# pweigmann/harmonic-power-flow

Hardware: AMD Instinct MI355X
Metric: NR iterations/sec + ms/iter, 1 000-bus x 25-harmonic feeder; |dV| vs reference (higher is better)
Workload: dtype f64

## Files before the change

### harmonic-power-flow_amd/csrc/hpf_block.hip

```cpp
#include <algorithm>
#include <chrono>
#include <complex>
#include <cstdio>
#include <cstdlib>
#include <rocsolver/rocsolver.h>
#include <thread>

#include "hpf_internal.hpp"
#include "hpf_gj.hpp"
#include "hpf_blk_jobs.hpp"
#include "hpf_blk_invert_mfma.hpp"
#include "hpf_gj_dense.hpp"
#include "hpf_gj_mfma.hpp"

using namespace hpf;

#ifdef HPF_FACTOR_STAMPS
#define HPF_STAMP_DECL long long st0 = 0, st1 = 0, st2 = 0, st3 = 0, st4 = 0, st5 = 0, st6 = 0
#define HPF_STAMP(v) \
    if (ablate & 16) v = __builtin_amdgcn_s_memtime()
#else
#define HPF_STAMP_DECL
#define HPF_STAMP(v)
#endif

namespace {

// ... 745 lines not shown
#endif
        const int i = bid - nb_sl - nb_lf;
        back_q_body<B>(i % n_gj, i / n_gj, M, T, gj_nodes, b, N, Nc, active, Zall, wall, xall, (double*)nullptr, Hall, Minv, lfK, lfS, s0);
    }
}

template <int B>
int launch_level_back(hpf_handle* h, const TreeDev& T, const int* sl_nodes, int n_sl, const int* lf_nodes, int n_lf, const int* gj_nodes, int n_gj,
                      const int* active) {
    const Tree& tr = active_tree(h);
    const unsigned ytiles = (unsigned)((h->cur_S + LB_SB - 1) / LB_SB);
#if HPF_BATCH_XCD
    const unsigned grid = (unsigned)(((n_sl + 7) / 8) * 8 + ((n_lf + 7) / 8) * 8) * ytiles + (unsigned)n_gj * (unsigned)h->cur_S;
#else
    const unsigned grid = (unsigned)(n_sl + n_lf) * ytiles + (unsigned)n_gj * (unsigned)h->cur_S;
#endif
    if ((unsigned)(n_sl + n_lf) * ytiles + (unsigned)n_gj * (unsigned)h->cur_S == 0) return HPF_OK;
    hipLaunchKernelGGL((k_level_back<B>), dim3(grid), dim3(256), 0, h->cur_stream, h->M, T, sl_nodes, n_sl, lf_nodes, n_lf, gj_nodes, n_gj, 2 * h->Hn,
                       h->N, h->Nc, active, h->cur_S, h->d_Z, h->d_w, h->d_x, h->d_H, tr.d_Minv, tr.d_lbimg, tr.d_sbimg, tr.d_lzimg, h->d_lfK, h->d_lfS,
                       h->cur_s0);
    return launch_status(h);
}

__global__ __launch_bounds__(256) void k_border_prepare(int n, int Hn, int Bst, int b, int r, int v0, int vfirst, const int* __restrict__ tb_bus,
                                                        int n_tb, const double* __restrict__ g, cplx* __restrict__ U, cplx* __restrict__ E,
                                                        cplx* __restrict__ I0, double* __restrict__ fb) {
    const int j = blockIdx.y, v = vfirst + j;
    const size_t dst = (size_t)(v0 + j);
    const int t = blockIdx.x * 256 + threadIdx.x;
    if (t < n * Hn) {
        U[dst * n * Hn + t] = U[(size_t)r * n * Hn + t];
        E[dst * n * Hn + t] = E[(size_t)r * n * Hn + t];
    }
    if (t < n) I0[dst * n + t] = I0[(size_t)r * n + t];
    if (t < n * Bst) {
        double val = 0.0;
        if (v == 0) {
            val = fb[(size_t)r * n * Bst + t];
            if (g) {
                const int bus = t / Bst, l = t - bus * Bst;
                if (l < b)
                    for (int a = 0; a < n_tb; ++a)
                        if (tb_bus[a] == bus) val -= g[a * b + l];
            }
        } else {
            const int a = (v - 1) / b, l = (v - 1) - a * b;
// ... 55 lines not shown
    if (h->gj_mode != 1 || !h->sw.fuse_levels || (BW != 12 && BW != 28 && BW != 52)) return false;
    return BW == 52 || level_batched(h, T, l, nullptr) > 0;
}

bool tree_levels_fused(hpf_handle* h) {
    if (h->solver != HPF_SOLVER_BLOCK_TREE) return false;
    const Tree& T = active_tree(h);
    const int BW = wave_block_size(2 * h->Hn);
    if (T.n_levels == 0) return false;
    for (int l = 0; l < T.n_levels; ++l)
        if (T.lvl_ptr[l + 1] > T.lvl_ptr[l] && !level_is_fused(h, T, l, BW)) return false;
    return true;
}

Tree& active_tree(hpf_handle* h) { return (h->has_ctree && h->gj_mode == 1) ? h->ctree : h->tree; }

static void tree_free_one(Tree& T);
static void tree_free_one_fwd(Tree& T) { tree_free_one(T); }
static void tree_free_one(Tree& T) {
    void* ptrs[] = {T.d_parent, T.d_lvl_nodes, T.d_dep_nodes, T.d_child_ptr, T.d_child, T.d_e_up, T.d_e_dn,
                    T.d_child_mid, T.d_lin, T.d_lin_ptr, T.d_lin_post, T.d_all_ptr, T.d_all_post, T.d_fdesc, T.d_child3,
                    T.d_bdesc, T.d_dchild, T.d_chain_ptr, T.d_chain_nodes, T.d_chain_ch, T.d_Minv, T.d_lrec, T.d_crec, T.d_cnode, T.d_arec,
                    T.d_lzrec, T.d_lzimg, T.d_lbimg, T.d_bleaf, T.d_bsleaf, T.d_bsleaf_dep, T.d_sbimg, T.d_lbrec, T.d_lbptr, T.d_lb2rec, T.d_lb2x, T.d_lb2ptr, T.d_lb2cptr, T.d_lb2clist,
                    T.d_comp_child};
    for (void* p : ptrs)
        if (p) hipFree(p);
}

void tree_free(hpf_handle* h) {
    tree_free_one(h->tree);
    tree_free_one(h->ctree);
    void* bp[] = {h->d_tb_bus, h->d_tb_ptr, h->d_tb_adj, h->d_bM, h->d_brhs, h->d_bipiv, h->d_binfo, h->d_bM0, h->d_brhs0,
                  h->d_sel_P, h->d_sel_pidx, h->d_sel_toff, h->d_sel_S, h->d_sel_Z, h->d_sel_Up, h->d_sel_W, h->d_sel_X, h->d_sel_tie, h->d_sel_jobs,
                  h->d_sel_hl, h->d_sel_slot, h->d_sel_cptr, h->d_sel_clist, h->d_sel_dw, h->d_bB, h->d_bgj_jobs,
                  h->d_sel_bM, h->d_sel_rhs, h->d_sel_g, h->d_sel_res, h->d_sel_info};
    for (void* q2 : bp)
        if (q2) hipFree(q2);
}

int tree_alloc_scenarios(hpf_handle* h) {
    const int bw = wave_block_size(2 * h->Hn);
    const size_t b = bw ? (size_t)bw : 2 * (size_t)h->Hn, S = h->S_alloc, n = h->n;
    hipError_t e;
    const size_t ct = bw ? (size_t)(((bw + 16) / 16) * ((bw + 16) / 16) * 256) : 0;
    if ((e = hipMalloc((void**)&h->d_Z, sizeof(double) * S * n * (b * b > ct ? b * b : ct))) != hipSuccess ||
        (e = hipMalloc((void**)&h->d_w, sizeof(double) * S * n * b)) != hipSuccess ||
        (e = hipMalloc((void**)&h->d_x, sizeof(double) * S * n * b)) != hipSuccess ||
// ... 175 lines not shown
            case 28: r = factor_level<28>(h, T, td, l, active); break;
            case 52: r = factor_level<52>(h, T, td, l, active); break;
            case 100:
                if (h->gj_mode == 1) {
                    r = launch_factor_q<100>(h, td, T.d_fdesc + FDESC * (size_t)T.lvl_ptr[l], cnt, active, T.lvl_all_leaf[l] != 0);
                    break;
                }
                [[fallthrough]];
            default: r = factor_level_generic(h, td, T.d_lvl_nodes + T.lvl_ptr[l], cnt, active);
        }
        if (r) return r;
    }
    return HPF_OK;
}

static bool back_is_fused(const hpf_handle* h, const Tree& T, int BW) {
    bool fused = h->sw.fuse_back && h->cur_S <= h->sw.fuse_back_max && h->sw.leafbatch && h->has_ctree && h->gj_mode == 1 && BW == 52 &&
                 (int)T.bsl_dep_ptr.size() == T.n_depths + 1 && (int)T.bleaf_dep_ptr.size() == T.n_depths + 1 && (int)T.dep_nleaf.size() >= T.n_depths;
    for (int dl = 1; fused && dl < T.n_depths; ++dl)
        fused = T.bsl_dep_ptr[dl + 1] - T.bsl_dep_ptr[dl] + T.bleaf_dep_ptr[dl + 1] - T.bleaf_dep_ptr[dl] == T.dep_nleaf[dl];
    return fused && T.bsl_dep_ptr[1] == 0 && T.bleaf_dep_ptr[1] == 0;
}

template <int BW>
static int back_depth(hpf_handle* h, const Tree& T, const TreeDev& td, int dl, int nlb, const int* active) {
    const int cnt = T.dep_ptr[dl + 1] - T.dep_ptr[dl];
    if (h->gj_mode != 1) return launch_back_w<BW>(h, td, T.d_dep_nodes + T.dep_ptr[dl], cnt, active);
    return cnt > nlb ? launch_back_q<BW>(h, td, T.d_bdesc + 4 * (size_t)(T.dep_ptr[dl] + nlb), cnt - nlb, active) : HPF_OK;
}

template <int BW>
static int back_batched(hpf_handle* h, const Tree& T, const int* active) {
    for (size_t gi = 0; gi + 1 < T.bsleaf_ptr.size() && T.n_bsleaf > 0; ++gi) {
        const int b0 = T.bsleaf_ptr[gi], cnt = T.bsleaf_ptr[gi + 1] - b0;
        if (cnt <= 0) continue;
        if (int r = launch_sleaf_back_batch<BW>(h, T.d_bsleaf + 8 * (size_t)b0, cnt, active)) return r;
    }
    return T.n_bleaf > 0 ? launch_leaf_back_batch<BW>(h, T.d_bleaf, T.n_bleaf, active) : HPF_OK;
}

static int back_sweep(hpf_handle* h, const Tree& T, const TreeDev& td, const int* active, int Bst) {
    ScopedTimer tb(h, T_BACK);
    const int BW = wave_block_size(2 * h->Hn);
    const bool fused_back = back_is_fused(h, T, BW);
    for (int dl = 0; dl < T.n_depths; ++dl) {
        const int cnt = T.dep_ptr[dl + 1] - T.dep_ptr[dl];
        if (cnt == 0) continue;
        const int* nodes = T.d_dep_nodes + T.dep_ptr[dl];
        const int nlb = (h->sw.leafbatch && h->has_ctree && dl > 0 && dl < (int)T.dep_nleaf.size()) ? T.dep_nleaf[dl] : 0;
        int r = HPF_OK;
        if (fused_back) {
            const int n_sl = dl > 0 ? T.bsl_dep_ptr[dl + 1] - T.bsl_dep_ptr[dl] : 0, n_lf = dl > 0 ? T.bleaf_dep_ptr[dl + 1] - T.bleaf_dep_ptr[dl] : 0;
            r = launch_level_back<52>(h, td, T.d_bsleaf_dep + 8 * (size_t)T.bsl_dep_ptr[dl], n_sl, T.d_bleaf + 4 * (size_t)T.bleaf_dep_ptr[dl], n_lf,
                                      T.d_bdesc + 4 * (size_t)(T.dep_ptr[dl] + nlb), cnt - nlb, active);
        } else {
            switch (BW) {
                case 12: r = back_depth<12>(h, T, td, dl, nlb, active); break;
                case 28: r = back_depth<28>(h, T, td, dl, nlb, active); break;
                case 52: r = back_depth<52>(h, T, td, dl, nlb, active); break;
                case 100:
                    if (h->gj_mode == 1) {
                        r = launch_back_q<100>(h, td, T.d_bdesc + 4 * (size_t)T.dep_ptr[dl], cnt, active);
                        break;
                    }
                    [[fallthrough]];
                default:
// ... 715 lines not shown
```

### harmonic-power-flow_amd/csrc/hpf_internal.hpp

```cpp
#pragma once
#include <hip/hip_runtime.h>
#include <rocblas/rocblas.h>
#include <stdint.h>

#include <stdlib.h>
#include <string.h>

#include <string>
#include <vector>

#include "../../include/hpf.h"
#include "hpf_assembly.hpp"
#include "hpf_switches.hpp"

namespace hpf {

enum LinForm {
    LIN_ROOTS = 0,
    LIN_BUNDLE,
    LIN_TREE,
    LIN_LEVELS
};

enum { T_MISMATCH = 0, T_JACOBIAN = 1, T_SOLVE = 2, T_UPDATE = 3, T_BACK = 4, T_GJ = 5, T_GJ_DEV = 6, T_COUNT = 7 };

struct TimedSpan {
    int which;
    hipEvent_t e0, e1;
};

struct Tree {
    int n_levels = 0;
    int n_depths = 0;
    std::vector<int> parent;
    std::vector<int> lvl_ptr;
    std::vector<int> lvl_nodes;
    std::vector<int> dep_ptr;
    std::vector<int> dep_nodes;
    std::vector<int> child_ptr;
    std::vector<int> child;
    std::vector<int> child_mid;
    std::vector<int> lin;
    std::vector<int> lin_ptr;
    std::vector<int> lin_post;
    std::vector<int> all_ptr, all_post;
    int n_lin_roots = 0;
    int n_dense = 0;
    int* d_parent = nullptr;
    int* d_lvl_nodes = nullptr;
    int* d_dep_nodes = nullptr;
    int* d_child_ptr = nullptr;
    int* d_child = nullptr;
// ... 33 lines not shown
    int* d_cnode = nullptr;
    int n_all_heights = 0;
    std::vector<int> ah_ptr;
    int* d_arec = nullptr;
    std::vector<int> lvl_all_leaf;
    std::vector<int> toff_tab;
    std::vector<char> plain_gj;
    int n_cleaf = 0;
    double* d_Minv = nullptr;
    int n_lazy_parents = 0, n_lazy_leaves = 0;
    int n_lazy_level0 = 0;
    std::vector<int> lvl_nbatch;
    std::vector<int> dep_nleaf;
    std::vector<int> dep_nskip;
    int census[8] = {0, 0, 0, 0, 0, 0, 0, 0};
    std::vector<int> bsleaf_ptr;
    int n_bsleaf = 0;
    int* d_bsleaf = nullptr;
    double* d_sbimg = nullptr;
    std::vector<int> bsl_dep_ptr, bleaf_dep_ptr;
    int* d_bsleaf_dep = nullptr;
    int n_bleaf = 0;
    int* d_bleaf = nullptr;
    double* d_lbimg = nullptr;
    int* d_lzrec = nullptr;
    double* d_lzimg = nullptr;
    int n_comp = 0;
    std::vector<int> comp_v, comp_c;
    int* d_comp_child = nullptr;
    double plan_ms = 0.0;
    double flops_per_solve = 0.0;
    double flops_factor = 0.0;
    double bytes_back = 0.0;
    double bytes_factor = 0.0;
    double flops_gj = 0.0, bytes_gj = 0.0;
    int n_gj_launches = 0;
};

}

struct hpf_handle {
    hpf::Switches sw;
    hpf::Model M{};
    int n = 0, m = 0, c = 0, Hn = 0, nnz = 0, n_dev = 0, coupled = 0, solver = 0, device = 0;
    int S_max = 0, S = 0;
    int S_alloc = 0;
// ... 169 lines not shown
```

### harmonic-power-flow_amd/csrc/hpf_quad.hpp

```cpp
#pragma once

template <int CTRL>
__device__ __forceinline__ double dpp_f64(double v) {
    int lo = __double2loint(v), hi = __double2hiint(v);
    lo = __builtin_amdgcn_update_dpp(lo, lo, CTRL, 0xf, 0xf, false);
    hi = __builtin_amdgcn_update_dpp(hi, hi, CTRL, 0xf, 0xf, false);
    return __hiloint2double(hi, lo);
}

__device__ __forceinline__ double row_sum16(double v) {
    v += dpp_f64<0xB1>(v);
    v += dpp_f64<0x4E>(v);
    v += dpp_f64<0x141>(v);
    v += dpp_f64<0x140>(v);
    return v;
}

__device__ __forceinline__ Blk2 blk_current(cplx y, cplx Uj, cplx Ej) {
    Blk2 b;
    b.dV = cmul_unf(y, Ej);
    b.dA = cmul_unf(cmulj(y), Uj);
    return b;
}
__device__ __forceinline__ Blk2 blk_current_diag(cplx y, cplx U, cplx E, cplx yn, bool nonlinear) {
// ... 1278 lines not shown
        __shared__ cplx ynl[(B / 2) * (B / 2)];
        __shared__ double tab[(B / 2) * 8], dgb[RP * 3], cc[NT][RP * 3], panel[2][NT * 64], wl[2][16], pv[2][16], gl[NT * 32], hl[NT * 32];
        __shared__ double slb[B <= 52 ? 2 * B * 10 + 200 + 4 : 1];
        lds.ynl = ynl; lds.tab = tab; lds.dgb = dgb; lds.cc = cc; lds.panel = panel; lds.wl = wl; lds.pv = pv; lds.gl = gl; lds.hl = hl; lds.slb = slb;
        lds.gl2 = lds.hl2 = lds.pbuf = nullptr;
    } else {
        __shared__ __attribute__((aligned(16))) double smem[factor_q_lds<B>()];
        lds = FqLds<B>::carve(smem);
    }
    int bx = blockIdx.x, by = blockIdx.y;
#if HPF_LEAF_XCD
    if constexpr (LEAF) {
        const unsigned id = blockIdx.x, t = id >> 3, S_ = gridDim.y == 1 ? leaf_S : 1u;
        by = (int)(t % S_);
        bx = (int)((t / S_) * 8u + (id & 7u));
        if (bx >= leaf_count) return;
    }
#endif
    factor_q_body<B, LEAF>(lds, bx, by, M, T, nodes, b, N, Nc, active, Uall, Eall, fall, Zall, wall, linAall, Call, Hall, I0all, chG,
                           chH, chD, chy, Minv, lfK, lfS, dbg, ablate, s0, pivflag, piv_limit, tstamp);
}

template <int B>
__device__ __forceinline__ void back_q_body(
    const int bx_, const int by_, const Model& M, const TreeDev& T, const int* __restrict__ nodes, int b, int N, int Nc, const int* __restrict__ active,
    const double* __restrict__ Zall, const double* __restrict__ wall, double* __restrict__ xall, double* __restrict__ step,
    const double* __restrict__ Hall, const double* __restrict__ Minv, const double* __restrict__ lfK,
    const double* __restrict__ lfS, int s0) {
    constexpr int NT = (B + 16) / 16;
    constexpr size_t CT = (size_t)NT * NT * 256;
    const int s = active ? active[by_ + s0] : (int)by_ + s0;
    if (s < 0) return;
    const int4 kp = reinterpret_cast<const int4*>(nodes)[bx_];
    const int k = kp.x, par = kp.y, cleaf = kp.z;
    const int crole = kp.w >> 28, cinfo = kp.w & 0x0fffffff;
    const int tid = threadIdx.x, lane = tid & 63, lg = lane >> 4, jj = lane & 15;
    const int wv = __builtin_amdgcn_readfirstlane(tid >> 6);
    const int n = M.n, c = M.c, Hn = M.Hn;
    double* xs = xall + (size_t)s * n * B;
    constexpr int RP = 16 * NT > 64 ? 16 * NT : 64;
    __shared__ double part[NT][RP];
    __shared__ double mcl[RP * 2], zl[RP];
    double x = 0.0;
    if (tid < B) x = wall[((size_t)s * n + k) * B + tid];
    if (par >= 0) {
        double zr[NT * 4];
        if (cleaf) {
            TileIO<B>::load(Minv + (size_t)(cleaf - 1) * CT, wv, lg, jj, zr);
        } else {
            TileIO<B>::load(Zall + ((size_t)s * n + k) * CT, wv, lg, jj, zr);
        }
        const int col = 16 * wv + jj, p = col >> 1, t1 = col & 1;
        double tv = 0.0;
        if (crole == 2) {
            double hr[NT * 4];
            TileIO<B>::load(T.cF + (((size_t)s * T.n_comp + cinfo) * 3 + 2) * CT, wv, lg, jj, hr);
            const double xpc = col < b ? xs[(size_t)par * B + col] : 0.0;
#pragma unroll
            for (int e = 0; e < NT * 4; ++e)
                if (16 * (e >> 2) + 4 * (e & 3) < B) {
                    const double r = row_sum16(hr[e] * xpc);
                    if (jj == 0) part[wv][16 * (e >> 2) + lg + 4 * (e & 3)] = r;
                }
            __syncthreads();
            if (tid < B) {
                double acc = part[0][tid];
#pragma unroll
                for (int w2 = 1; w2 < NT; ++w2) acc += part[w2][tid];
                zl[tid] = acc;
            }
            __syncthreads();
            tv = col < b ? zl[col] : 0.0;
            __syncthreads();
        } else if (col < b) {
            const double* hk = Hall + ((size_t)s * n + k) * Hn * 4 + p * 4 + t1 * 2;
            const double* xp = xs + (size_t)par * B;
            tv = fma(hk[1], xp[2 * p + 1], hk[0] * xp[2 * p]);
            if (crole == 1) {
                const double* h2 = T.cH2 + ((size_t)s * T.n_comp + cinfo) * Hn * 4 + p * 4 + t1 * 2;
                const double* xc = xs + (size_t)T.comp_child[cinfo] * B;
                tv += fma(h2[1], xc[2 * p + 1], h2[0] * xc[2 * p]);
            }
        }
        if (cleaf && tid < 2) zl[tid] = tv;
        const double tvs = (cleaf && col < 2) ? 0.0 : tv;
        __builtin_amdgcn_sched_barrier(0);
#pragma unroll
        for (int e = 0; e < NT * 4; ++e)
            if (16 * (e >> 2) + 4 * (e & 3) < B) {
                const double r = row_sum16(zr[e] * tvs);
                if (jj == 0) part[wv][16 * (e >> 2) + lg + 4 * (e & 3)] = r;
                if (cleaf && wv == 0 && jj < 2) mcl[(16 * (e >> 2) + lg + 4 * (e & 3)) * 2 + jj] = zr[e];
            }
        __syncthreads();
        double acc = 0.0;
        if (tid < B) {
            acc = part[0][tid];
#pragma unroll
            for (int w2 = 1; w2 < NT; ++w2) acc += part[w2][tid];
        }
        if (cleaf) {
            double t0 = 0.0, t1v = 0.0;
            if (tid < B) {
                t0 = zl[0];
                t1v = zl[1];
            }
            __syncthreads();
            if (tid < 2) zl[tid] = acc + (tid == 0 ? t0 : t1v);
            __syncthreads();
            if (tid < B) {
                const double* kk = lfK + ((size_t)s * n + k) * 12;
                const double u0 = fma(kk[1], zl[1], kk[0] * zl[0]), u1 = fma(kk[3], zl[1], kk[2] * zl[0]);
                const double c0r = tid < 2 ? (tid == 0 ? 1.0 : 0.0) : mcl[tid * 2];
                const double c1r = tid < 2 ? (tid == 1 ? 1.0 : 0.0) : mcl[tid * 2 + 1];
                acc = fma(c1r, u1, fma(c0r, u0, tid < 2 ? 0.0 : acc));
            }
            __syncthreads();
            if (tid < B) zl[tid] = acc;
            __syncthreads();
            if (tid < B) {
                const double* si = lfS + (((size_t)s * n + k) * Hn + (tid >> 1)) * 4 + 2 * (tid & 1);
                acc = (tid >> 1) < Hn ? fma(si[1], zl[tid | 1], si[0] * zl[tid & ~1]) : acc;
            }
        }
        if (tid < B) x -= acc;
    }
    if (tid < B) {
        xs[(size_t)k * B + tid] = x;
        if (step && tid < b) {
            const int kst = (tid >> 1) * n + k;
            double* st = step + (size_t)s * N;
            if (tid & 1) {
                if (kst >= c) st[Nc + kst - c] = x;
            } else {
                if (kst >= 1) st[kst - 1] = x;
            }
        }
    }
}

template <int B>
__global__ __launch_bounds__(64 * ((B + 16) / 16)) void k_back_q(
    Model M, TreeDev T, const int* __restrict__ nodes, int b, int N, int Nc, const int* __restrict__ active,
    const double* __restrict__ Zall, const double* __restrict__ wall, double* __restrict__ xall, double* __restrict__ step,
    const double* __restrict__ Hall, const double* __restrict__ Minv, const double* __restrict__ lfK,
    const double* __restrict__ lfS, int s0) {
    back_q_body<B>(blockIdx.x, blockIdx.y, M, T, nodes, b, N, Nc, active, Zall, wall, xall, step, Hall, Minv, lfK, lfS, s0);
}

// ... 31 lines not shown
```

### harmonic-power-flow_amd/csrc/hpf_switches.hpp

```cpp
#pragma once
#include <stdlib.h>
#include <string.h>

#include <string>

namespace hpf {

struct Switches {
    bool tree_info = false;
    bool border_info = false;
    bool queue_info = false;
    std::string tree_dump;
    int debug_ablate = 0;
    int gj_mode = 1;
    int n_groups = 4;
    bool leafbatch = true;
    bool fuse_levels = true;
    bool fuse_back = true;
    int fuse_back_max = 32;
    int border_slot_cap = 1024;
    bool lintree = true;
    bool linbundle = true;
    bool chainbundle = true;
    int sleaf = 2;
    bool slback = true;
    bool sllazy = true;
    bool slnest = true;
    int lazy = 2;
    bool compress = true;
    bool mesh_sel = true;
    int border_gj = 96;
    bool border_gj_mfma = true;
    double border_pivlim = 1e3;
    double mesh_batch_gb = 48.0;
    bool mesh_batch_gb_given = false;
};

inline Switches parse_switches(const char* options, bool env_opt_in) {
    const std::string opts = options ? options : "";
    auto find = [&](const char* name) -> const char* {
        const size_t ln = strlen(name);
        size_t pos = 0;
// ... 3 lines not shown
            pos += ln;
        }
        return env_opt_in ? getenv(name) : nullptr;
    };
    auto flag = [&](const char* name, bool& f) {
        if (const char* v = find(name)) f = atoi(v) != 0;
    };
    auto integer = [&](const char* name, int& f) {
        if (const char* v = find(name)) f = atoi(v);
    };
    Switches s;
    s.tree_info = find("HPF_TREE_INFO") != nullptr;
    s.border_info = find("HPF_BORDER_INFO") != nullptr;
    s.queue_info = find("HPF_QUEUE_INFO") != nullptr;
    if (env_opt_in)
        if (const char* v = getenv("HPF_TREE_DUMP")) s.tree_dump = v;
    integer("HPF_DEBUG_ABLATE", s.debug_ablate);
    if (const char* v = find("HPF_GJ_MODE")) s.gj_mode = atoi(v) ? 1 : 0;
    if (const char* v = find("HPF_GROUPS")) s.n_groups = atoi(v) < 1 ? 1 : (atoi(v) > 8 ? 8 : atoi(v));
    flag("HPF_LEAFBATCH", s.leafbatch);
    flag("HPF_FUSELEVEL", s.fuse_levels);
    flag("HPF_FUSEBACK", s.fuse_back);
    integer("HPF_FUSEBACK_MAX", s.fuse_back_max);
    integer("HPF_BORDER_SLOTS", s.border_slot_cap);
    flag("HPF_LINTREE", s.lintree);
    flag("HPF_LINBUNDLE", s.linbundle);
    flag("HPF_CHAINBUNDLE", s.chainbundle);
    integer("HPF_SLEAF", s.sleaf);
    flag("HPF_SLBACK", s.slback);
    flag("HPF_SLLAZY", s.sllazy);
    flag("HPF_SLNEST", s.slnest);
    integer("HPF_LAZY", s.lazy);
    flag("HPF_COMPRESS", s.compress);
    flag("HPF_MESH_SEL", s.mesh_sel);
    integer("HPF_BORDER_GJ", s.border_gj);
    flag("HPF_BORDER_GJ_MFMA", s.border_gj_mfma);
    if (const char* v = find("HPF_BORDER_PIVLIM"))
        if (atof(v) > 0.0) s.border_pivlim = atof(v);
    if (const char* v = find("HPF_MESH_BATCH_GB")) {
        s.mesh_batch_gb = atof(v);
        s.mesh_batch_gb_given = true;
    }
    return s;
}

inline bool env_switches_opted_in() {
// ... 6 lines not shown
```

### harmonic-power-flow_amd/csrc/hpf_tree_plan.hpp

```cpp
#pragma once

#if defined(__x86_64__) && !defined(__HIP_DEVICE_COMPILE__)
__attribute__((target("avx2"))) static void cplx_row_axpy_avx2(double* __restrict__ rr, double* __restrict__ ri, const double* __restrict__ cr,
                                                                const double* __restrict__ ci, double fr, double fi, int nn) {
    for (int c2 = 0; c2 < nn; ++c2) {
        rr[c2] -= fr * cr[c2] - fi * ci[c2];
        ri[c2] -= fr * ci[c2] + fi * cr[c2];
    }
}
#endif
static unsigned host_threads() {
    if (const char* e = getenv("HPF_HOST_THREADS")) return atoi(e) < 1 ? 1u : (unsigned)atoi(e);
    const unsigned hw = std::thread::hardware_concurrency();
    return hw < 1 ? 1u : (hw > 16 ? 16u : hw);
}
static void cplx_row_axpy(double* __restrict__ rr, double* __restrict__ ri, const double* __restrict__ cr, const double* __restrict__ ci,
                          double fr, double fi, int nn) {
#if defined(__x86_64__) && !defined(__HIP_DEVICE_COMPILE__)
    static const bool has_avx2 = __builtin_cpu_supports("avx2");
    if (has_avx2) {
        cplx_row_axpy_avx2(rr, ri, cr, ci, fr, fi, nn);
        return;
    }
#endif
    for (int c2 = 0; c2 < nn; ++c2) {
        rr[c2] -= fr * cr[c2] - fi * ci[c2];
        ri[c2] -= fr * ci[c2] + fi * cr[c2];
    }
}

namespace hpf {

static void tree_free_one_fwd(Tree& T);
static int tree_build_into(hpf_handle* h, const hpf_desc* d, Tree& T, bool contract) {
    const auto t_begin = std::chrono::steady_clock::now();
    const int n = d->n;
    const int b = 2 * d->Hn;
    if (b > 16 * 7) return HPF_E_ARG;
    if (d->nnz != n + 2 * (n - 1) + 2 * h->n_ties) return HPF_E_TOPOLOGY;
    T.parent.assign(n, -2);
    std::vector<int> order, depth(n, 0), height(n, 0), e_up(n, -1), e_dn(n, -1);
    order.reserve(n);
    order.push_back(0);
    T.parent[0] = -1;
    for (size_t oi = 0; oi < order.size(); ++oi) {
        const int i = order[oi];
        for (int e = d->rowptr[i]; e < d->rowptr[i + 1]; ++e) {
            const int j = d->col[e];
            if (j == i) continue;
            if (T.parent[j] == -2) {
                T.parent[j] = i;
                e_dn[j] = e;
                order.push_back(j);
            }
// ... 1058 lines not shown
            if (sb_ord[k] >= 0) r[14] |= 8;
            r[34] = sl_slot[k];
            r[35] = (int)(sl_base + sl_off[k]);
            r[39] = sb_ord[k] >= 0 ? sb_ord[k] : 0;
        }
        for (int i = 40; i < FDESC; ++i) r[i] = 0;
        if (comp_role[k]) {
            r[40] = comp_role[k];
            r[41] = comp_idx[k];
            if (comp_role[k] == 1) {
                const int cb = comp_child[k];
                r[42] = cb;
                r[43] = e_dn[cb];
                r[44] = e_up[cb];
                r[45] = pass[T.parent[cb]] ? 1 : 0;
            }
        }
        const int kb = T.dep_nodes[pos];
        bdesc[(size_t)pos * 4 + 0] = kb;
        bdesc[(size_t)pos * 4 + 1] = pard[kb];
        bdesc[(size_t)pos * 4 + 2] = cleaf_of[kb] + 1;
        bdesc[(size_t)pos * 4 + 3] = comp_role[kb] ? ((comp_role[kb] << 28) | comp_idx[kb]) : 0;
    }
    {
        int nc = 0, nb = 0, nn = 0;
        for (int i = 0; i < n; ++i) {
            if (!kept(i)) continue;
            if (cleaf_of[i] >= 0) ++nc;
            if (sl_off[i] >= 0 && lz_idx[i] >= 0) {
                ++nb;
                if (sl_nest[i] > 0) ++nn;
            }
        }
        const int cs[8] = {T.n_dense, T.n_dense - nc - nb, nc, T.n_lazy_leaves, nb, nn, T.n_levels, T.n_depths};
        for (int i = 0; i < 8; ++i) T.census[i] = cs[i];
    }
    const double bd = b;
    T.flops_factor = 0.0;
    T.bytes_factor = 0.0;
    T.bytes_back = 0.0;
    int n_dense_nonroot = 0;
    const int BWf = wave_block_size(b);
    const int NTf = (BWf + 16) / 16, LWf = (BWf + 1 - 16 * (NTf - 1)) <= 8 ? 8 : 16;
    const double TB = BWf ? (double)((BWf + 3) / 4) * ((NTf - 1) * 64 + 4 * LWf) * 8.0 : 8.0 * bd * bd;
    T.flops_gj = 0.0;
    T.bytes_gj = 0.0;
// ... 58 lines not shown
                (i >= d->m ? sl_nl : sl_lin)++;
                sl_lvl[height[i] < 3 ? height[i] : 3]++;
            }
        fprintf(stderr, "hpf tree: buses whose dense children are all lazy leaves: %d nonlinear + %d linear (levels 1/2/3+: %d/%d/%d), %d built as super-leaves\n",
                sl_nl, sl_lin, sl_lvl[1], sl_lvl[2], sl_lvl[3], n_sleaf);
    }
    if (h->sw.tree_info)
        fprintf(stderr, "hpf tree (%s): %d buses, %d dense in %d levels, %d chains, %d constant-inverse leaves, %d lazy under %d parents\n",
                contract ? "contracted" : "plain", n, T.n_dense, T.n_levels, T.n_chains, T.n_cleaf, T.n_lazy_leaves, T.n_lazy_parents);
    if (const char* dump_path = h->plan_path ? h->plan_path : (h->sw.tree_dump.empty() ? nullptr : h->sw.tree_dump.c_str())) {
        if (FILE* fp = fopen(dump_path, contract ? "w" : "a")) {
            h->plan_written = true;
            fprintf(fp, "# %s tree: k pard height depth kind(0 gauss-jordan, 1 constant-inverse leaf, 2 bordered) vector_only hbm_children via_chain compress_role "
                        "plain_gauss_jordan_on_a_root_path_of_a_tie_endpoint\n", contract ? "contracted" : "plain");
            if (h->n_ties > 0)
                fprintf(fp, "# meshed: %d loop-closing lines, %d endpoint buses, border %d unknowns, bordered step %s\n", h->n_ties, h->n_tb, h->m_border,
                        h->mesh_sel ? "factor-once" : "virtual sweeps");
            for (int pos = 0; pos < T.n_dense; ++pos) {
                const int k = T.lvl_nodes[pos];
                const int kind = cleaf_of[k] >= 0 ? 1 : ((sl_off[k] >= 0 && lz_idx[k] >= 0) ? 2 : 0);
                fprintf(fp, "%d %d %d %d %d %d %d %d %d %d\n", k, pard[k], height[k], depth[k], kind, is_lazy[k],
                        dchild_ptr[k + 1] - dchild_ptr[k] - n_lazy[k] - n_slz[k], (k > 0 && pass[T.parent[k]]) ? 1 : 0, comp_role[k],
                        (use_fp && fmask[k]) ? (T.plain_gj[k] ? 1 : -1) : 0);
            }
            fclose(fp);
        }
    }
    T.plan_ms = std::chrono::duration<double, std::milli>(std::chrono::steady_clock::now() - t_begin).count();
    if (h->sw.tree_info) fprintf(stderr, "hpf tree (%s): planned on the host in %.1f ms\n", contract ? "contracted" : "plain", T.plan_ms);
    if (h->plan_only) return HPF_OK;
    int r;
    if ((r = upload(h, &T.d_parent, T.parent))) return r;
    if ((r = upload(h, &T.d_lvl_nodes, T.lvl_nodes))) return r;
    if ((r = upload(h, &T.d_dep_nodes, T.dep_nodes))) return r;
    if ((r = upload(h, &T.d_child_ptr, T.child_ptr))) return r;
    if ((r = upload(h, &T.d_child, T.child))) return r;
    if ((r = upload(h, &T.d_e_up, e_up))) return r;
    if ((r = upload(h, &T.d_e_dn, e_dn))) return r;
    if ((r = upload(h, &T.d_child_mid, T.child_mid))) return r;
    if ((r = upload(h, &T.d_lin, T.lin))) return r;
    if ((r = upload(h, &T.d_lin_ptr, T.lin_ptr))) return r;
    if ((r = upload(h, &T.d_lin_post, T.lin_post))) return r;
    if ((r = upload(h, &T.d_all_ptr, T.all_ptr))) return r;
    if ((r = upload(h, &T.d_all_post, T.all_post))) return r;
    if ((r = upload(h, &T.d_fdesc, fdesc))) return r;
    if ((r = upload(h, &T.d_child3, child3))) return r;
// ... 18 lines not shown
        T.bsl_dep_ptr.assign(1, 0);
        for (int dl = 0; dl < T.n_depths; ++dl) {
            for (int pos = T.dep_ptr[dl]; pos < T.dep_ptr[dl + 1]; ++pos) {
                const int kb = T.dep_nodes[pos];
                if (sb_ord[kb] < 0 || sl_off[kb] < 0 || lz_idx[kb] < 0) continue;
                const int rec[8] = {kb, pard[kb], sb_ord[kb], (int)(sl_base + sl_off[kb]), sb_m[kb], 0, 0, 0};
                bsd.insert(bsd.end(), rec, rec + 8);
            }
            T.bsl_dep_ptr.push_back((int)bsd.size() / 8);
        }
        if ((r = upload(h, &T.d_bsleaf_dep, bsd))) return r;
        if ((r = upload(h, &T.d_sbimg, sbimg))) return r;
    }
    {
        std::vector<int> bleaf;
        T.bleaf_dep_ptr.assign(1, 0);
        for (int dl = 0; dl < T.n_depths; ++dl) {
            for (int pos = T.dep_ptr[dl]; pos < T.dep_ptr[dl + 1]; ++pos)
                if (bdesc[(size_t)pos * 4 + 2] > 0 && bdesc[(size_t)pos * 4 + 1] >= 0) bleaf.insert(bleaf.end(), &bdesc[(size_t)pos * 4], &bdesc[(size_t)pos * 4] + 4);
            T.bleaf_dep_ptr.push_back((int)bleaf.size() / 4);
        }
        T.n_bleaf = (int)bleaf.size() / 4;
        if ((r = upload(h, &T.d_bleaf, bleaf))) return r;
    }
    if ((r = upload(h, &T.d_dchild, dchild))) return r;
    if ((r = upload(h, &T.d_comp_child, T.comp_c))) return r;
    if ((r = upload(h, &T.d_chain_ptr, T.chain_ptr))) return r;
    if ((r = upload(h, &T.d_chain_nodes, T.chain_nodes))) return r;
    if ((r = upload(h, &T.d_chain_ch, T.chain_ch))) return r;
    if ((r = upload(h, &T.d_Minv, minv))) return r;
    if ((r = upload(h, &T.d_lzrec, lzrec))) return r;
    if ((r = upload(h, &T.d_lzimg, lzimg))) return r;
    if ((r = upload(h, &T.d_lbimg, lbimg))) return r;
    if ((r = upload(h, &T.d_lrec, lrec))) return r;
    if ((r = upload(h, &T.d_lb2rec, lb2rec))) return r;
    if ((r = upload(h, &T.d_lb2x, lb2x))) return r;
    if ((r = upload(h, &T.d_lb2ptr, lb2ptr))) return r;
    if ((r = upload(h, &T.d_lb2cptr, lb2cptr))) return r;
    if ((r = upload(h, &T.d_lb2clist, lb2clist))) return r;
    if ((r = upload(h, &T.d_lbrec, lbrec))) return r;
    if ((r = upload(h, &T.d_lbptr, lbptr))) return r;
    if ((r = upload(h, &T.d_crec, crec))) return r;
    if ((r = upload(h, &T.d_cnode, cnode))) return r;
    if ((r = upload(h, &T.d_arec, arec))) return r;
    return HPF_OK;
}
// ... 27 lines not shown
```

Measured before the change: 147,000.

## Walk top tree portion in one kernel per subtree unit instead of per-depth launches

Adds a back-substitution 'walk' kernel in which each block processes a whole unit of tree nodes (a root path plus a subtree) sequentially, keeping parent solutions in shared memory. The next node's operands are prefetched while the current one is reduced. A host planner partitions the non-leaf part of the contracted tree into units capped at 32 nodes, and the remaining batched leaf stages run as a few level launches. The goal is to replace many per-depth kernel launches with one, at the cost of redundant recomputation of shared path nodes across units and more serial work inside each block.

```diff
diff --git a/harmonic-power-flow_amd/csrc/hpf_block.hip b/harmonic-power-flow_amd/csrc/hpf_block.hip
--- a/harmonic-power-flow_amd/csrc/hpf_block.hip
+++ b/harmonic-power-flow_amd/csrc/hpf_block.hip
@@ -3,6 +3,7 @@
 #include <complex>
 #include <cstdio>
 #include <cstdlib>
+#include <functional>
 #include <rocsolver/rocsolver.h>
 #include <thread>
 
@@ -794,6 +795,53 @@
     return launch_status(h);
 }
 
+template <int B>
+__global__ __launch_bounds__(256) void k_back_walk(
+    Model M, TreeDev T, const int2* __restrict__ wunit, const int* __restrict__ wrec, int n_units, int b, const int* __restrict__ active, int S_cnt,
+    const double* __restrict__ Zall, const double* __restrict__ wall, double* __restrict__ xall, const double* __restrict__ Hall,
+    const double* __restrict__ Minv, const double* __restrict__ lfK, const double* __restrict__ lfS, int s0) {
+    static_assert(64 * ((B + 16) / 16) == 256, "k_back_walk: blocks of 52 rows (four wavefronts)");
+    const int id = (int)blockIdx.x, t_ = id >> 3;
+    const int u = t_ % n_units, sl = (t_ / n_units) * 8 + (id & 7);
+    if (sl >= S_cnt) return;
+    const int s = active ? active[sl + s0] : sl + s0;
+    if (s < 0) return;
+    const int tid = threadIdx.x;
+    __shared__ int4 rec[WALK_MAX][2];
+    __shared__ double xw[WALK_MAX][B];
+    const int2 ur = wunit[u];
+    const int len = ur.y;
+    if (tid < 2 * len) rec[tid >> 1][tid & 1] = reinterpret_cast<const int4*>(wrec)[2 * (size_t)ur.x + tid];
+    __syncthreads();
+    auto uni = [](int4 v) {
+        return int4{__builtin_amdgcn_readfirstlane(v.x), __builtin_amdgcn_readfirstlane(v.y), __builtin_amdgcn_readfirstlane(v.z),
+                    __builtin_amdgcn_readfirstlane(v.w)};
+    };
+    double* xs = xall + (size_t)s * M.n * B;
+    BackQIn<B> cur, nxt;
+    back_q_load<B>(uni(rec[0][0]), s, M, T, b, Zall, wall, Hall, Minv, cur);
+    for (int i = 0; i < len; ++i) {
+        const int4 kp = uni(rec[i][0]), sp = uni(rec[i][1]);
+        if (i + 1 < len) back_q_load<B>(uni(rec[i + 1][0]), s, M, T, b, Zall, wall, Hall, Minv, nxt);
+        const double x = back_q_reduce<B>(kp, s, M, b, cur, xw[sp.x >= 0 ? sp.x : 0], xw[sp.y >= 0 ? sp.y : 0], lfK, lfS);
+        if (tid < B) {
+            xw[i][tid] = x;
+            if (sp.z) xs[(size_t)kp.x * B + tid] = x;
+        }
+        __syncthreads();
+        cur = nxt;
+    }
+}
+
+template <int B>
+int launch_back_walk(hpf_handle* h, const Tree& tr, const TreeDev& T, const int* active) {
+    const unsigned grid = (unsigned)tr.n_wunits * (unsigned)((h->cur_S + 7) / 8) * 8u;
+    if (grid == 0) return HPF_OK;
+    hipLaunchKernelGGL((k_back_walk<B>), dim3(grid), dim3(256), 0, h->cur_stream, h->M, T, (const int2*)tr.d_wunit, tr.d_wrec, tr.n_wunits,
+                       2 * h->Hn, active, h->cur_S, h->d_Z, h->d_w, h->d_x, h->d_H, tr.d_Minv, h->d_lfK, h->d_lfS, h->cur_s0);
+    return launch_status(h);
+}
+
 __global__ __launch_bounds__(256) void k_border_prepare(int n, int Hn, int Bst, int b, int r, int v0, int vfirst, const int* __restrict__ tb_bus,
                                                         int n_tb, const double* __restrict__ g, cplx* __restrict__ U, cplx* __restrict__ E,
                                                         cplx* __restrict__ I0, double* __restrict__ fb) {
@@ -895,7 +943,7 @@
                     T.d_child_mid, T.d_lin, T.d_lin_ptr, T.d_lin_post, T.d_all_ptr, T.d_all_post, T.d_fdesc, T.d_child3,
                     T.d_bdesc, T.d_dchild, T.d_chain_ptr, T.d_chain_nodes, T.d_chain_ch, T.d_Minv, T.d_lrec, T.d_crec, T.d_cnode, T.d_arec,
                     T.d_lzrec, T.d_lzimg, T.d_lbimg, T.d_bleaf, T.d_bsleaf, T.d_bsleaf_dep, T.d_sbimg, T.d_lbrec, T.d_lbptr, T.d_lb2rec, T.d_lb2x, T.d_lb2ptr, T.d_lb2cptr, T.d_lb2clist,
-                    T.d_comp_child};
+                    T.d_comp_child, T.d_wunit, T.d_wrec, T.d_wsl, T.d_wlf};
     for (void* p : ptrs)
         if (p) hipFree(p);
 }
@@ -1117,6 +1165,21 @@
     return fused && T.bsl_dep_ptr[1] == 0 && T.bleaf_dep_ptr[1] == 0;
 }
 
+static bool back_is_walked(const hpf_handle* h, const Tree& T, int BW) {
+    return h->sw.back_walk && T.n_wunits > 0 && back_is_fused(h, T, BW);
+}
+
+static int back_walk(hpf_handle* h, const Tree& T, const TreeDev& td, const int* active) {
+    if (int r = launch_back_walk<52>(h, T, td, active)) return r;
+    for (int st = 0; st < T.n_wstages; ++st) {
+        const int n_sl = T.wsl_ptr[st + 1] - T.wsl_ptr[st], n_lf = T.wlf_ptr[st + 1] - T.wlf_ptr[st];
+        if (int r = launch_level_back<52>(h, td, T.d_wsl + 8 * (size_t)T.wsl_ptr[st], n_sl, T.d_wlf + 4 * (size_t)T.wlf_ptr[st], n_lf,
+                                          (const int*)nullptr, 0, active))
+            return r;
+    }
+    return HPF_OK;
+}
+
 template <int BW>
 static int back_depth(hpf_handle* h, const Tree& T, const TreeDev& td, int dl, int nlb, const int* active) {
     const int cnt = T.dep_ptr[dl + 1] - T.dep_ptr[dl];
@@ -1137,6 +1200,10 @@
 static int back_sweep(hpf_handle* h, const Tree& T, const TreeDev& td, const int* active, int Bst) {
     ScopedTimer tb(h, T_BACK);
     const int BW = wave_block_size(2 * h->Hn);
+    if (back_is_walked(h, T, BW)) {
+        if (int r = back_walk(h, T, td, active)) return r;
+        return lin_back(h, T, td, active, Bst);
+    }
     const bool fused_back = back_is_fused(h, T, BW);
     for (int dl = 0; dl < T.n_depths; ++dl) {
         const int cnt = T.dep_ptr[dl + 1] - T.dep_ptr[dl];
diff --git a/harmonic-power-flow_amd/csrc/hpf_internal.hpp b/harmonic-power-flow_amd/csrc/hpf_internal.hpp
--- a/harmonic-power-flow_amd/csrc/hpf_internal.hpp
+++ b/harmonic-power-flow_amd/csrc/hpf_internal.hpp
@@ -28,6 +28,8 @@
     int which;
     hipEvent_t e0, e1;
 };
+
+constexpr int WALK_MAX = 32;
 
 struct Tree {
     int n_levels = 0;
@@ -107,6 +109,14 @@
     int* d_bsleaf_dep = nullptr;
     int n_bleaf = 0;
     int* d_bleaf = nullptr;
+    int n_wunits = 0, walk_cap = 0, walk_longest = 0, walk_entries = 0;
+    std::vector<int> wunit_ptr;
+    int* d_wunit = nullptr;
+    int* d_wrec = nullptr;
+    int n_wstages = 0;
+    std::vector<int> wsl_ptr, wlf_ptr;
+    int* d_wsl = nullptr;
+    int* d_wlf = nullptr;
     double* d_lbimg = nullptr;
     int* d_lzrec = nullptr;
     double* d_lzimg = nullptr;
diff --git a/harmonic-power-flow_amd/csrc/hpf_quad.hpp b/harmonic-power-flow_amd/csrc/hpf_quad.hpp
--- a/harmonic-power-flow_amd/csrc/hpf_quad.hpp
+++ b/harmonic-power-flow_amd/csrc/hpf_quad.hpp
@@ -1324,44 +1324,72 @@
 }
 
 template <int B>
-__device__ __forceinline__ void back_q_body(
-    const int bx_, const int by_, const Model& M, const TreeDev& T, const int* __restrict__ nodes, int b, int N, int Nc, const int* __restrict__ active,
-    const double* __restrict__ Zall, const double* __restrict__ wall, double* __restrict__ xall, double* __restrict__ step,
-    const double* __restrict__ Hall, const double* __restrict__ Minv, const double* __restrict__ lfK,
-    const double* __restrict__ lfS, int s0) {
+struct BackQIn {
+    static constexpr int NT = (B + 16) / 16;
+    double x;
+    double zr[NT * 4];
+    double hr[NT * 4];
+    double hk0, hk1;
+    double h20, h21;
+};
+
+template <int B>
+__device__ __forceinline__ void back_q_load(const int4 kp, const int s, const Model& M, const TreeDev& T, int b, const double* __restrict__ Zall,
+                                            const double* __restrict__ wall, const double* __restrict__ Hall, const double* __restrict__ Minv,
+                                            BackQIn<B>& in) {
     constexpr int NT = (B + 16) / 16;
     constexpr size_t CT = (size_t)NT * NT * 256;
-    const int s = active ? active[by_ + s0] : (int)by_ + s0;
-    if (s < 0) return;
-    const int4 kp = reinterpret_cast<const int4*>(nodes)[bx_];
     const int k = kp.x, par = kp.y, cleaf = kp.z;
     const int crole = kp.w >> 28, cinfo = kp.w & 0x0fffffff;
     const int tid = threadIdx.x, lane = tid & 63, lg = lane >> 4, jj = lane & 15;
     const int wv = __builtin_amdgcn_readfirstlane(tid >> 6);
-    const int n = M.n, c = M.c, Hn = M.Hn;
-    double* xs = xall + (size_t)s * n * B;
+    const int n = M.n, Hn = M.Hn;
+    in.x = 0.0;
+    if (tid < B) in.x = wall[((size_t)s * n + k) * B + tid];
+    if (par < 0) return;
+    if (cleaf) {
+        TileIO<B>::load(Minv + (size_t)(cleaf - 1) * CT, wv, lg, jj, in.zr);
+    } else {
+        TileIO<B>::load(Zall + ((size_t)s * n + k) * CT, wv, lg, jj, in.zr);
+    }
+    const int col = 16 * wv + jj, p = col >> 1, t1 = col & 1;
+    if (crole == 2) {
+        TileIO<B>::load(T.cF + (((size_t)s * T.n_comp + cinfo) * 3 + 2) * CT, wv, lg, jj, in.hr);
+    } else if (col < b) {
+        const double* hk = Hall + ((size_t)s * n + k) * Hn * 4 + p * 4 + t1 * 2;
+        in.hk0 = hk[0];
+        in.hk1 = hk[1];
+        if (crole == 1) {
+            const double* h2 = T.cH2 + ((size_t)s * T.n_comp + cinfo) * Hn * 4 + p * 4 + t1 * 2;
+            in.h20 = h2[0];
+            in.h21 = h2[1];
+        }
+    }
+}
+
+template <int B>
+__device__ __forceinline__ double back_q_reduce(const int4 kp, const int s, const Model& M, int b, const BackQIn<B>& in,
+                                                const double* xp, const double* xc, const double* __restrict__ lfK,
+                                                const double* __restrict__ lfS) {
+    constexpr int NT = (B + 16) / 16;
+    const int k = kp.x, par = kp.y, cleaf = kp.z;
+    const int crole = kp.w >> 28;
+    const int tid = threadIdx.x, lane = tid & 63, lg = lane >> 4, jj = lane & 15;
+    const int wv = __builtin_amdgcn_readfirstlane(tid >> 6);
+    const int n = M.n, Hn = M.Hn;
     constexpr int RP = 16 * NT > 64 ? 16 * NT : 64;
     __shared__ double part[NT][RP];
     __shared__ double mcl[RP * 2], zl[RP];
-    double x = 0.0;
-    if (tid < B) x = wall[((size_t)s * n + k) * B + tid];
+    double x = in.x;
     if (par >= 0) {
-        double zr[NT * 4];
-        if (cleaf) {
-            TileIO<B>::load(Minv + (size_t)(cleaf - 1) * CT, wv, lg, jj, zr);
-        } else {
-            TileIO<B>::load(Zall + ((size_t)s * n + k) * CT, wv, lg, jj, zr);
-        }
-        const int col = 16 * wv + jj, p = col >> 1, t1 = col & 1;
+        const int col = 16 * wv + jj, p = col >> 1;
         double tv = 0.0;
         if (crole == 2) {
-            double hr[NT * 4];
-            TileIO<B>::load(T.cF + (((size_t)s * T.n_comp + cinfo) * 3 + 2) * CT, wv, lg, jj, hr);
-            const double xpc = col < b ? xs[(size_t)par * B + col] : 0.0;
+            const double xpc = col < b ? xp[col] : 0.0;
 #pragma unroll
             for (int e = 0; e < NT * 4; ++e)
                 if (16 * (e >> 2) + 4 * (e & 3) < B) {
-                    const double r = row_sum16(hr[e] * xpc);
+                    const double r = row_sum16(in.hr[e] * xpc);
                     if (jj == 0) part[wv][16 * (e >> 2) + lg + 4 * (e & 3)] = r;
                 }
             __syncthreads();
@@ -1375,14 +1403,8 @@
             tv = col < b ? zl[col] : 0.0;
             __syncthreads();
         } else if (col < b) {
-            const double* hk = Hall + ((size_t)s * n + k) * Hn * 4 + p * 4 + t1 * 2;
-            const double* xp = xs + (size_t)par * B;
-            tv = fma(hk[1], xp[2 * p + 1], hk[0] * xp[2 * p]);
-            if (crole == 1) {
-                const double* h2 = T.cH2 + ((size_t)s * T.n_comp + cinfo) * Hn * 4 + p * 4 + t1 * 2;
-                const double* xc = xs + (size_t)T.comp_child[cinfo] * B;
-                tv += fma(h2[1], xc[2 * p + 1], h2[0] * xc[2 * p]);
-            }
+            tv = fma(in.hk1, xp[2 * p + 1], in.hk0 * xp[2 * p]);
+            if (crole == 1) tv += fma(in.h21, xc[2 * p + 1], in.h20 * xc[2 * p]);
         }
         if (cleaf && tid < 2) zl[tid] = tv;
         const double tvs = (cleaf && col < 2) ? 0.0 : tv;
@@ -1390,9 +1412,9 @@
 #pragma unroll
         for (int e = 0; e < NT * 4; ++e)
             if (16 * (e >> 2) + 4 * (e & 3) < B) {
-                const double r = row_sum16(zr[e] * tvs);
+                const double r = row_sum16(in.zr[e] * tvs);
                 if (jj == 0) part[wv][16 * (e >> 2) + lg + 4 * (e & 3)] = r;
-                if (cleaf && wv == 0 && jj < 2) mcl[(16 * (e >> 2) + lg + 4 * (e & 3)) * 2 + jj] = zr[e];
+                if (cleaf && wv == 0 && jj < 2) mcl[(16 * (e >> 2) + lg + 4 * (e & 3)) * 2 + jj] = in.zr[e];
             }
         __syncthreads();
         double acc = 0.0;
@@ -1427,6 +1449,26 @@
         }
         if (tid < B) x -= acc;
     }
+    return x;
+}
+
+template <int B>
+__device__ __forceinline__ void back_q_body(
+    const int bx_, const int by_, const Model& M, const TreeDev& T, const int* __restrict__ nodes, int b, int N, int Nc, const int* __restrict__ active,
+    const double* __restrict__ Zall, const double* __restrict__ wall, double* __restrict__ xall, double* __restrict__ step,
+    const double* __restrict__ Hall, const double* __restrict__ Minv, const double* __restrict__ lfK,
+    const double* __restrict__ lfS, int s0) {
+    const int s = active ? active[by_ + s0] : (int)by_ + s0;
+    if (s < 0) return;
+    const int4 kp = reinterpret_cast<const int4*>(nodes)[bx_];
+    const int k = kp.x, par = kp.y;
+    const int tid = threadIdx.x;
+    const int n = M.n, c = M.c;
+    double* xs = xall + (size_t)s * n * B;
+    BackQIn<B> in;
+    back_q_load<B>(kp, s, M, T, b, Zall, wall, Hall, Minv, in);
+    const double* xc = (kp.w >> 28) == 1 ? xs + (size_t)T.comp_child[kp.w & 0x0fffffff] * B : xs;
+    const double x = back_q_reduce<B>(kp, s, M, b, in, xs + (size_t)(par >= 0 ? par : 0) * B, xc, lfK, lfS);
     if (tid < B) {
         xs[(size_t)k * B + tid] = x;
         if (step && tid < b) {
diff --git a/harmonic-power-flow_amd/csrc/hpf_switches.hpp b/harmonic-power-flow_amd/csrc/hpf_switches.hpp
--- a/harmonic-power-flow_amd/csrc/hpf_switches.hpp
+++ b/harmonic-power-flow_amd/csrc/hpf_switches.hpp
@@ -18,6 +18,8 @@
     bool fuse_levels = true;
     bool fuse_back = true;
     int fuse_back_max = 32;
+    bool back_walk = true;
+    int back_walk_cap = 0;
     int border_slot_cap = 1024;
     bool lintree = true;
     bool linbundle = true;
@@ -67,6 +69,8 @@
     flag("HPF_FUSELEVEL", s.fuse_levels);
     flag("HPF_FUSEBACK", s.fuse_back);
     integer("HPF_FUSEBACK_MAX", s.fuse_back_max);
+    flag("HPF_BACKWALK", s.back_walk);
+    integer("HPF_BACKWALK_CAP", s.back_walk_cap);
     integer("HPF_BORDER_SLOTS", s.border_slot_cap);
     flag("HPF_LINTREE", s.lintree);
     flag("HPF_LINBUNDLE", s.linbundle);
diff --git a/harmonic-power-flow_amd/csrc/hpf_tree_plan.hpp b/harmonic-power-flow_amd/csrc/hpf_tree_plan.hpp
--- a/harmonic-power-flow_amd/csrc/hpf_tree_plan.hpp
+++ b/harmonic-power-flow_amd/csrc/hpf_tree_plan.hpp
@@ -30,6 +30,113 @@
 }
 
 namespace hpf {
+
+static bool plan_back_walk(Tree& T, const std::vector<int>& bdesc, const std::vector<int>& comp_child, const std::vector<char>& in_walk,
+                           int n, int cap_sw, std::vector<int>& wunit, std::vector<int>& wrec) {
+    std::vector<int> wpar(n, -1), wd(n, 0), sz(n, 0), pos_of(n, -1), kids_ptr(n + 1, 0), kids, order;
+    for (int pos = 0; pos < T.n_dense; ++pos) {
+        const int k = bdesc[(size_t)pos * 4];
+        if (!in_walk[k]) continue;
+        pos_of[k] = pos;
+        const int role = bdesc[(size_t)pos * 4 + 3] >> 28;
+        const int q = role == 1 ? comp_child[k] : bdesc[(size_t)pos * 4 + 1];
+        if (q >= 0 && (!in_walk[q] || pos_of[q] < 0)) return false;
+        wpar[k] = q;
+        wd[k] = q >= 0 ? wd[q] + 1 : 0;
+        if (role == 1) {
+            const int p = bdesc[(size_t)pos * 4 + 1];
+            int a = q;
+            while (a >= 0 && a != p) a = wpar[a];
+            if (a != p) return false;
+        }
+        order.push_back(k);
+    }
+    if (order.empty()) return false;
+    int lmin = 0;
+    for (int k : order) lmin = std::max(lmin, wd[k] + 1);
+    if (lmin > WALK_MAX) return false;
+    const int cap = std::min(WALK_MAX, std::max(lmin, cap_sw > 0 ? cap_sw : (3 * lmin + 1) / 2));
+    for (int k : order)
+        if (wpar[k] >= 0) kids_ptr[wpar[k] + 1]++;
+    for (int i = 0; i < n; ++i) kids_ptr[i + 1] += kids_ptr[i];
+    kids.resize(kids_ptr[n]);
+    {
+        std::vector<int> fill(kids_ptr.begin(), kids_ptr.end() - 1);
+        for (int k : order)
+            if (wpar[k] >= 0) kids[fill[wpar[k]]++] = k;
+    }
+    for (auto it = order.rbegin(); it != order.rend(); ++it) {
+        sz[*it] += 1;
+        if (wpar[*it] >= 0) sz[wpar[*it]] += sz[*it];
+    }
+    auto fits = [&](int k) { return wd[k] + sz[k] <= cap; };
+    std::vector<std::vector<int>> units;
+    std::function<void(int, std::vector<int>&)> preorder = [&](int k, std::vector<int>& out) {
+        out.push_back(k);
+        for (int i = kids_ptr[k]; i < kids_ptr[k + 1]; ++i) preorder(kids[i], out);
+    };
+    std::function<void(int)> cut = [&](int u) {
+        std::vector<int> path;
+        for (int a = u; a >= 0; a = wpar[a]) path.push_back(a);
+        std::reverse(path.begin(), path.end());
+        if (fits(u)) {
+            path.pop_back();
+            units.push_back(path);
+            preorder(u, units.back());
+            return;
+        }
+        std::vector<int> fit;
+        for (int i = kids_ptr[u]; i < kids_ptr[u + 1]; ++i)
+            if (fits(kids[i])) fit.push_back(kids[i]);
+        std::stable_sort(fit.begin(), fit.end(), [&](int a, int c2) { return sz[a] > sz[c2]; });
+        const size_t first = units.size();
+        for (int c2 : fit) {
+            size_t ui = first;
+            while (ui < units.size() && units[ui].size() + sz[c2] > (size_t)cap) ++ui;
+            if (ui == units.size()) units.push_back(path);
+            preorder(c2, units[ui]);
+        }
+        for (int i = kids_ptr[u]; i < kids_ptr[u + 1]; ++i)
+            if (!fits(kids[i])) cut(kids[i]);
+    };
+    for (int k : order)
+        if (wpar[k] < 0) cut(k);
+    std::vector<char> owned(n, 0);
+    std::vector<int> idx(units.size());
+    for (size_t i = 0; i < units.size(); ++i) idx[i] = (int)i;
+    std::stable_sort(idx.begin(), idx.end(), [&](int a, int c2) { return units[a].size() > units[c2].size(); });
+    std::vector<std::vector<char>> own(units.size());
+    for (size_t ui = 0; ui < units.size(); ++ui) {
+        own[ui].assign(units[ui].size(), 0);
+        for (size_t i = 0; i < units[ui].size(); ++i)
+            if (!owned[units[ui][i]]) owned[units[ui][i]] = own[ui][i] = 1;
+    }
+    wunit.clear();
+    wrec.clear();
+    std::vector<int> slot(n, -1);
+    for (int ui : idx) {
+        const std::vector<int>& U = units[ui];
+        wunit.push_back((int)wrec.size() / 8);
+        wunit.push_back((int)U.size());
+        for (size_t i = 0; i < U.size(); ++i) {
+            const int k = U[i], pos = pos_of[k];
+            slot[k] = (int)i;
+            const int par = bdesc[(size_t)pos * 4 + 1], role = bdesc[(size_t)pos * 4 + 3] >> 28;
+            const int rec[8] = {k, par, bdesc[(size_t)pos * 4 + 2], bdesc[(size_t)pos * 4 + 3], par >= 0 ? slot[par] : -1,
+                                role == 1 ? slot[comp_child[k]] : -1, own[ui][i], 0};
+            if ((par >= 0 && rec[4] < 0) || (role == 1 && rec[5] < 0)) return false;
+            wrec.insert(wrec.end(), rec, rec + 8);
+        }
+        for (int k : U) slot[k] = -1;
+    }
+    for (int k : order)
+        if (!owned[k]) return false;
+    T.n_wunits = (int)units.size();
+    T.walk_cap = cap;
+    T.walk_longest = (int)units[idx[0]].size();
+    T.walk_entries = (int)wrec.size() / 8;
+    return true;
+}
 
 static void tree_free_one_fwd(Tree& T);
 static int tree_build_into(hpf_handle* h, const hpf_desc* d, Tree& T, bool contract) {
@@ -1134,6 +1241,50 @@
         bdesc[(size_t)pos * 4 + 2] = cleaf_of[kb] + 1;
         bdesc[(size_t)pos * 4 + 3] = comp_role[kb] ? ((comp_role[kb] << 28) | comp_idx[kb]) : 0;
     }
+    std::vector<int> wunit, wrec, wsl, wlf;
+    T.n_wunits = T.n_wstages = 0;
+    if (contract && BWc == 52 && h->sw.back_walk && h->sw.leafbatch && T.n_depths > 0) {
+        std::vector<char> in_walk(n, 0), is_bsl(n, 0), is_blf(n, 0);
+        bool ok = (int)T.dep_nleaf.size() >= T.n_depths;
+        for (int dl = 0; ok && dl < T.n_depths; ++dl)
+            for (int pos = T.dep_ptr[dl]; pos < T.dep_ptr[dl + 1]; ++pos) {
+                const int kb = T.dep_nodes[pos];
+                if (dl == 0 || pos >= T.dep_ptr[dl] + T.dep_nleaf[dl]) in_walk[kb] = 1;
+                else if (cleaf_of[kb] >= 0 && pard[kb] >= 0) is_blf[kb] = 1;
+                else if (sb_ord[kb] >= 0 && sl_off[kb] >= 0 && lz_idx[kb] >= 0) is_bsl[kb] = 1;
+                else ok = false;
+            }
+        std::vector<int> stage(n, -1);
+        int nst = 0;
+        for (int pos = 0; ok && pos < T.n_dense; ++pos) {
+            const int kb = T.dep_nodes[pos], p = pard[kb];
+            if (in_walk[kb]) continue;
+            stage[kb] = p < 0 ? -1 : (in_walk[p] ? 0 : (is_bsl[p] ? stage[p] + 1 : -1));
+            if (stage[kb] < 0) ok = false;
+            nst = std::max(nst, stage[kb] + 1);
+        }
+        if (ok && plan_back_walk(T, bdesc, comp_child, in_walk, n, h->sw.back_walk_cap, wunit, wrec)) {
+            T.n_wstages = nst;
+            T.wsl_ptr.assign(1, 0);
+            T.wlf_ptr.assign(1, 0);
+            for (int st = 0; st < nst; ++st) {
+                for (int pos = 0; pos < T.n_dense; ++pos) {
+                    const int kb = T.dep_nodes[pos];
+                    if (stage[kb] != st) continue;
+                    if (is_bsl[kb]) {
+                        const int rec[8] = {kb, pard[kb], sb_ord[kb], (int)(sl_base + sl_off[kb]), sb_m[kb], 0, 0, 0};
+                        wsl.insert(wsl.end(), rec, rec + 8);
+                    } else {
+                        wlf.insert(wlf.end(), &bdesc[(size_t)pos * 4], &bdesc[(size_t)pos * 4] + 4);
+                    }
+                }
+                T.wsl_ptr.push_back((int)wsl.size() / 8);
+                T.wlf_ptr.push_back((int)wlf.size() / 4);
+            }
+        } else {
+            T.n_wunits = 0;
+        }
+    }
     {
         int nc = 0, nb = 0, nn = 0;
         for (int i = 0; i < n; ++i) {
@@ -1238,6 +1389,28 @@
                 fprintf(fp, "%d %d %d %d %d %d %d %d %d %d\n", k, pard[k], height[k], depth[k], kind, is_lazy[k],
                         dchild_ptr[k + 1] - dchild_ptr[k] - n_lazy[k] - n_slz[k], (k > 0 && pass[T.parent[k]]) ? 1 : 0, comp_role[k],
                         (use_fp && fmask[k]) ? (T.plain_gj[k] ? 1 : -1) : 0);
+            }
+            if (T.n_wunits > 0) {
+                int lin_l = T.chain_launches ? 1 : 0, dep_l = 0;
+                if (T.lin_form == LIN_LEVELS) {
+                    for (int hh = 0; hh < T.n_lin_heights; ++hh) lin_l += T.lh_ptr[hh + 1] > T.lh_ptr[hh];
+                } else {
+                    lin_l += T.lin_form != LIN_ROOTS || T.n_lin_roots > 0;
+                }
+                for (int dl = 0; dl < T.n_depths; ++dl) dep_l += T.dep_ptr[dl + 1] > T.dep_ptr[dl];
+                fprintf(fp, "# walk: cap %d, units %d, longest %d, buses walked %d, batched stages %d, back launches %d (per depth: %d)\n", T.walk_cap,
+                        T.n_wunits, T.walk_longest, T.walk_entries, T.n_wstages, 1 + T.n_wstages + lin_l, dep_l + lin_l);
+                fprintf(fp, "# walk compress (v c):");
+                for (int i = 0; i < T.n_comp; ++i) fprintf(fp, " %d %d", T.comp_v[i], T.comp_c[i]);
+                fprintf(fp, "\n");
+                for (int u = 0; u < T.n_wunits; ++u) {
+                    fprintf(fp, "# walk unit %d:", u);
+                    for (int i = 0; i < wunit[2 * u + 1]; ++i) {
+                        const int* rec = &wrec[(size_t)(wunit[2 * u] + i) * 8];
+                        fprintf(fp, " %d%s", rec[0], rec[6] ? "*" : "");
+                    }
+                    fprintf(fp, "\n");
+                }
             }
             fclose(fp);
         }
@@ -1302,6 +1475,12 @@
         }
         T.n_bleaf = (int)bleaf.size() / 4;
         if ((r = upload(h, &T.d_bleaf, bleaf))) return r;
+    }
+    if (T.n_wunits > 0) {
+        if ((r = upload(h, &T.d_wunit, wunit))) return r;
+        if ((r = upload(h, &T.d_wrec, wrec))) return r;
+        if ((r = upload(h, &T.d_wsl, wsl))) return r;
+        if ((r = upload(h, &T.d_wlf, wlf))) return r;
     }
     if ((r = upload(h, &T.d_dchild, dchild))) return r;
     if ((r = upload(h, &T.d_comp_child, T.comp_c))) return r;
```

Result: no change. 146,800 (median of 5 runs) (-0.1%).
